# eldar/deepcut-cnn

Measured on AMD Instinct MI355X. Metric: images/sec, DeeperCut ResNet-152 FCN forward (prob+loc_pred+next_pred), whole node, higher is better.
Workload: dtype f32

## Files before the change

### deepcut-cnn_amd/csrc/c_api.cpp

```cpp
#include <hip/hip_runtime_api.h>

#include <cstdio>
#include <cstring>
#include <memory>
#include <string>
#include <vector>

#include "../../include/deepcut_hip.h"
#include "net.h"

using namespace dc;


namespace {
thread_local std::string g_err;
int fail(int code, const std::string& msg) {
  g_err = msg;
  return code;
}
template <typename F>
int guard(F&& f) {
  try {
    f();
    return DC_OK;
// ... 526 lines not shown
const char* dc_net_debug_info(dc_net* net) {
  if (!net) return nullptr;
  Net* n = N(net);
  int rc = guard([&] { n->text_buf = n->debug_info_text(); });
  return rc == DC_OK ? n->text_buf.c_str() : nullptr;
}

const char* dc_net_tune_report(dc_net* net) {
  if (!net) return nullptr;
  Net* n = N(net);
  int rc = guard([&] { n->text_buf = n->tune_report_text(); });
  return rc == DC_OK ? n->text_buf.c_str() : nullptr;
}
int dc_net_set_tile(dc_net* net, const char* signature, const char* tile) {
  REQUIRE(net);
  REQUIRE(signature);
  REQUIRE(tile);
  return guard([&] { N(net)->set_tile(signature, tile); });
}

int dc_conv_variant_count(void) { return dc::conv_num_variants(); }
const char* dc_conv_variant_name(int i) { return i >= 0 && i < dc::conv_num_variants() ? dc::conv_variant(i).name : nullptr; }
int dc_conv_variant_esize(int i) { return i >= 0 && i < dc::conv_num_variants() ? dc::conv_variant_esize(i) : 0; }
int dc_conv_bf16_variant_count(void) { return dc::conv_num_bf16_variants(); }
const char* dc_conv_bf16_variant_name(int i) {
  return i >= 0 && i < dc::conv_num_bf16_variants() ? dc::conv_variant(dc::kBf16Variant0 + i).name : nullptr;
}
int dc_wino_half_pack(const float* g, int cout, int cin, int rowscale, float* out, float* row_scale) {
  REQUIRE(g);
  REQUIRE(out);
  REQUIRE(row_scale);
  if (cout <= 0 || cin <= 0 || cout % 32 || cin % 16) return fail(DC_EINVAL, "dc_wino_half_pack: cout must be a multiple of 32, cin of 16");
  return guard([&] { dc::wino_half_pack_filters(g, cout, cin, rowscale != 0, out, row_scale); });
}

int dc_stream1x1_pack(const float* g, int cout, int k, float* out) {
  if (!g || !out) return fail(DC_EINVAL, "dc_stream1x1_pack: null pointer");
  if (cout <= 0 || k <= 0 || cout % 32 || k % 16) return fail(DC_EINVAL, "dc_stream1x1_pack: cout must be a multiple of 32, k of 16");
  return guard([&] { dc::stream1x1_pack_filters(g, cout, k, out); });
}

int dc_stream1x1f_pack(const float* g, int cout, int k, float* out) {
  if (!g || !out) return fail(DC_EINVAL, "dc_stream1x1f_pack: null pointer");
  if (cout <= 0 || k <= 0 || cout % 16 || k % 16) return fail(DC_EINVAL, "dc_stream1x1f_pack: cout and k must be multiples of 16");
  return guard([&] { dc::stream1x1f_pack_filters(g, cout, k, out); });
}

int dc_stem7x7_pack(const float* g, int c, float* out) {
  if (!g || !out) return fail(DC_EINVAL, "dc_stem7x7_pack: null pointer");
  if (c < 1 || c > 4) return fail(DC_EINVAL, "dc_stem7x7_pack: 1 to 4 input channels");
  return guard([&] { dc::stem7x7_pack_filters(g, c, out); });
}

namespace {
inline NetGroup* G(dc_group* g) { return reinterpret_cast<NetGroup*>(g); }
}
int dc_group_create(dc_net* const* nets, int n, dc_group** out) {
  REQUIRE(nets);
  REQUIRE(out);
  *out = nullptr;
  if (n <= 0) return fail(DC_EINVAL, "a group needs at least one net");
  return guard([&] {
    std::vector<Net*> m;
    for (int i = 0; i < n; ++i) m.push_back(N(nets[i]));
    *out = reinterpret_cast<dc_group*>(NetGroup::create(m));
  });
// ... 138 lines not shown
```

### deepcut-cnn_amd/csrc/kernels.h

```cpp
#pragma once
#include <cstddef>
#include <cstdint>
#include <string>

namespace dc {

constexpr int kMaxTaps = 32;

void dc_magic(unsigned d, unsigned (&mg)[2]);

enum ElemKind { kElemF32 = 0, kElemF16 = 1, kElemBF16 = 2 };
inline int elem_kind_size(int kind) { return kind == kElemF32 ? 4 : 2; }
inline const char* elem_kind_name(int kind) { return kind == kElemF16 ? "f16" : kind == kElemBF16 ? "bf16" : "f32"; }

constexpr int kMaxClasses = 4;
struct ConvClass {
  int nty, ntx, dy0, ddy, x0, ddx, Ktot, x_bias;
  int OH, OW, M;
  int tiles_m;
  unsigned div_ohw[2];
  unsigned div_ow[2];
  long w_off;
  long y_off;
};
// ... 71 lines not shown
};
struct ConvMultiArgs {
  ConvGemmParams p;
  ConvMultiTable t;
};
static_assert(sizeof(ConvMultiArgs) <= 4096, "HIP kernel arguments are limited to 4 KB");

struct ConvVariant {
  const char* name;
  int BM, BN, WR, WC, WK;
};
int conv_num_variants();
const ConvVariant& conv_variant(int i);
int conv_variant_bk(int i);
int conv_variant_esize(int i);
constexpr int kBf16Variant0 = 2000;
int conv_num_bf16_variants();
inline bool is_bf16_variant(int v) { return v >= kBf16Variant0 && v < kBf16Variant0 + conv_num_bf16_variants(); }
int conv_variant_ekind(int v);
bool conv_variant_exists(int v);
const int* conv_variants_of(int ekind, int* count);
int conv_variant_by_name(const char* name);
bool conv_variant_multiclass(int i);
long conv_grid(const ConvGemmParams& p, int variant);
int launch_conv_gemm(const ConvGemmParams& p, int variant, void* stream);
long prepare_conv_multi(ConvGemmParams& p, ConvMultiTable& table, int nprob, int variant);
bool conv_variant_multiproblem(int i);
int launch_conv_multi(const ConvMultiArgs& a, int variant, long grid, void* stream);

bool wino_eligible(const ConvGemmParams& p);
bool wino_same3x3(const ConvGemmParams& p);
ConvGemmParams wino_launch_params(const ConvGemmParams& p, long grid, int bty, int btx, int blocks_per_wg);
long wino_grid(const ConvGemmParams& p);
size_t wino_packed_floats(int Cout, int Cin);
void wino_pack_filters(const float* g, int Cout, int Cin, float* out);
bool wino_half_eligible(const ConvGemmParams& p);
long wino_half_grid(const ConvGemmParams& p);
size_t wino_half_packed_elems(int Cout, int Cin);
void wino_half_pack_filters(const float* g, int Cout, int Cin, bool rowscale, float* out, float* row_scale);
int launch_wino_half(const ConvGemmParams& p, void* stream);
bool stream1x1_eligible(const ConvGemmParams& p);
long stream1x1_grid(const ConvGemmParams& p);
size_t stream1x1_packed_elems(int Cout, int K);
void stream1x1_pack_filters(const float* g, int Cout, int K, float* out);
int launch_stream1x1(const ConvGemmParams& p, void* stream);
bool stream1x1f_eligible(const ConvGemmParams& p);
long stream1x1f_grid(const ConvGemmParams& p);
size_t stream1x1f_packed_elems(int Cout, int K);
void stream1x1f_pack_filters(const float* g, int Cout, int K, float* out);
int launch_stream1x1f(const ConvGemmParams& p, void* stream);
bool stem_ws_eligible(const ConvGemmParams& p);
long stem_ws_grid(const ConvGemmParams& p);
size_t stem_ws_packed_elems();
void stem_ws_pack_filters(const float* rowtap, float* out);
int launch_stem_ws(const ConvGemmParams& p, void* stream);
bool stem7x7_eligible(const ConvGemmParams& p);
long stem7x7_grid(const ConvGemmParams& p);
size_t stem7x7_packed_elems();
void stem7x7_pack_filters(const float* g, int C, float* out);
int launch_stem7x7(const ConvGemmParams& p, void* stream);
long stream1x1_prepare_multi(const ConvGemmParams& p, const ConvMultiTable& tb, int nprob);
int launch_stream1x1_multi(const ConvMultiArgs& a, void* stream);

constexpr int kWinoVariant = 1000;
constexpr int kWinoVariant16 = 1001;
constexpr int kWinoHalf = 1002;
constexpr int kStreamHalf = 1003;
constexpr int kStemHalf = 1004;
constexpr int kStreamFloat = 1005;
constexpr int kStemFloat = 1006;
constexpr int kFormVariant0 = kWinoVariant, kNumForms = 7;
enum FormGeometry { kForm3x3, kForm1x1, kFormStem };
struct ConvForm {
  int variant;
  const char *name, *label;
  int ekind, geometry, waves;
  const char* const* timing_slots;
  bool (*eligible)(const ConvGemmParams& p);
  long (*grid)(const ConvGemmParams& p);
  int (*launch)(const ConvGemmParams& p, void* stream);
  bool own_scale;
  bool merges;
  long (*prepare_multi)(const ConvGemmParams& p, const ConvMultiTable& tb, int nprob);
  int (*launch_multi)(const ConvMultiArgs& a, void* stream);
  int sibling;
  const char* env;
};
const ConvForm* conv_form(int variant);

const char* variant_name(int v);
int variant_by_name(const char* name);
std::string variant_kernel_label(int v);
long variant_grid(const ConvGemmParams& p, int v);
int launch_conv(const ConvGemmParams& p, int v, void* stream);


int launch_maxpool(const void* x, void* y, int ekind, int NB, int H, int W, int C, int OH, int OW, int k, int s,
                   int pad, void* stream);

int launch_eltwise(const void* x, const void* z, const float* a, const float* b, void* y, int ekind, long total, int C,
                   int relu, int sigmoid, void* stream);

int launch_crop(const void* x, void* y, int ekind, int NB, int H, int W, int C, int oh, int ow, int OH, int OW,
                void* stream);

int launch_nchw_to_nhwc(const float* src, void* dst, int ekind, int NB, int C, int H, int W, int CP, void* stream);
int launch_nhwc_to_nchw(const void* src, void* dst, int ekind, int NB, int C, int H, int W, int CP, int c0,
                        void* stream, int dst_esize = 4);
int launch_f32_to_f16(const float* src, void* dst, long n, void* stream);
int launch_f32_to_bf16(const float* src, void* dst, long n, void* stream);

int launch_part_select(const void* prob, int pcp, int pc0, const void* loc, int lcp, int lc0, int ekind, int NB, int H, int W, int J, float thr,
                       int radius, double scale, int max_det, unsigned long long* spill, int* counts, double* out, void* stream);
int launch_pairwise_decode(const void* next, int ncp, int nc0, int ekind, int NB, int H, int W, int E, double scale, int ndet,
                           const int* det , const double* mean, const double* stdev, double* out,
                           void* stream);

struct ImagePrepParams {
  const unsigned char* src;
// ... 49 lines not shown
```

### deepcut-cnn_amd/csrc/kernels.hip

```cpp
#include <hip/hip_runtime.h>

#include <algorithm>
#include <cstdlib>
#include <cstring>
#include <type_traits>
#include <vector>

#include "kernel_prims.h"
#include "kernels.h"

namespace dc {


#define DC_KARG_TOUCH(n0, n1, n2, n3, n4)                                                                                  \
  unsigned n0, n1, n2, n3, n4;                                                                                             \
  {                                                                                                                        \
    const auto* ka_ = __builtin_amdgcn_kernarg_segment_ptr();                                                              \
    asm volatile("s_load_dword %0, %5, 0x0\n\ts_load_dword %1, %5, 0x40\n\ts_load_dword %2, %5, 0x80\n\ts_load_dword %3, %5, 0xc0\n\t" \
                 "s_load_dword %4, %5, 0x100"                                                                              \
                 : "=&s"(n0), "=&s"(n1), "=&s"(n2), "=&s"(n3), "=&s"(n4)                                                     \
                 : "s"(ka_));                                                                                              \
  }
#define DC_KARG_HOLD(n0, n1, n2, n3, n4) asm volatile("" ::"s"(n0), "s"(n1), "s"(n2), "s"(n3), "s"(n4))
static_assert(sizeof(ConvGemmParams) >= 0x140, "DC_KARG_TOUCH reads five 64-byte lines of the argument block");
// ... 1259 lines not shown
  const long blk = mc_xcd_grid(p, rows, nprob, tn, wtot, atot);
  if (blk <= 0 || blk > 0x7fffffffL) return -1;
  {
    const int lgx = p.mc_lgx, lgy = 3 - lgx;
    const unsigned w0 = (unsigned)(tn >> lgx);
    dc_magic(std::max(w0, 1u), p.div_rw[0]);
    dc_magic(w0 + 1, p.div_rw[1]);
    for (int qy = 0; qy < 8; ++qy) {
      int run = 0;
      for (int c = 0; c < kMaxProblems; ++c) {
        if (c < nprob && qy < (8 >> lgx)) {
          run += (int)((((long)tb.prob[c].tiles_m * (qy + 1)) >> lgy) - (((long)tb.prob[c].tiles_m * qy) >> lgy));
          tb.end[qy][c] = run;
        } else {
          tb.end[qy][c] = 0x7fffffff;
        }
      }
    }
  }
  return blk;
}

int launch_conv_multi(const ConvMultiArgs& a, int variant, long grid, void* stream) {
  if (const ConvForm* f = conv_form(variant)) return f->launch_multi ? f->launch_multi(a, stream) : (int)hipErrorInvalidValue;
  if (!dc_variant_ok(variant) || !entry_of(variant).kernel_mp || a.p.nprob < 1 || grid <= 0) return (int)hipErrorInvalidValue;
  const VariantEntry& e = entry_of(variant);
  const int nt = e.v.WR * e.v.WC * e.v.WK * 64;
  hipLaunchKernelGGL(e.kernel_mp, dim3((unsigned)grid), dim3(nt), 0, (hipStream_t)stream, a);
  return (int)hipGetLastError();
}

namespace {
constexpr int WBTY = 4, WBTX = 8, WBN = 16, WKC = 32;
constexpr int WRH = 2 * WBTY + 2, WRW = 2 * WBTX + 2;
constexpr int WPSTR = WKC + 4;
constexpr int WPITCH = 672;
constexpr int WSTAGE = WRH * WPITCH + 8;
constexpr int WNTH = 512;
static_assert(WPITCH >= WRW * WPSTR && (2 * WPITCH) % 64 == 0 && WPSTR == 36, "conflict-free ds_read_b128 layout (see above)");
static_assert(WPITCH % 4 == 0 && WPSTR % 4 == 0 && WSTAGE % 4 == 0, "16-byte units");
__device__ __forceinline__ int wino_rowbase(int row) { return row * WPITCH; }
__device__ __forceinline__ f32x2 wlo(f32x4 v) { return __builtin_shufflevector(v, v, 0, 1); }
__device__ __forceinline__ f32x2 whi(f32x4 v) { return __builtin_shufflevector(v, v, 2, 3); }
}

template <int NG>
__global__ __launch_bounds__(WNTH * NG, 4) void wino_f23_kernel(const ConvGemmParams p) {
  constexpr int NTH = WNTH * NG;
  constexpr int WNLD = (WRH * WRW * (WKC / 4) + NTH - 1) / NTH;
  const long long t_entry = (long long)__builtin_amdgcn_s_memrealtime();
  DC_KARG_TOUCH(ka0, ka1, ka2, ka3, ka4);
  __shared__ __attribute__((aligned(16))) float stage[3][WSTAGE];
  float (*part)[4][2][2][4][64] = reinterpret_cast<float (*)[4][2][2][4][64]>(&stage[0][0]);
  static_assert(sizeof(float) * NG * 4 * 2 * 2 * 4 * 64 <= sizeof(stage), "partials must fit in the staging ring");
  static_assert(2 * sizeof(stage) <= 160 * 1024, "two workgroups per CU");
  const int t = threadIdx.x, lane = t & 63, wave = t >> 6;
  auto stamp = [&](int slot) {
    if (p.dbg && lane == 0) {
      long long* d = p.dbg + ((long)blockIdx.x * (8 * NG) + wave) * 12;
      d[slot] = (long long)__builtin_readcyclecounter();
      if (slot == 0) d[8] = t_entry, d[10] = (long long)__builtin_amdgcn_s_memrealtime();
      if (slot == 7) d[9] = (long long)__builtin_amdgcn_s_memrealtime();
    }
  };
  stamp(0);
  const int C = p.klen, H = p.x_rows, W = p.x_rowlen / p.klen;
  const int d = p.ddy;
  const int NBY = p.w_NBY, NBX = p.w_NBX;
  const int nblk = p.w_nblk;
  int lb = blockIdx.x;
  if (p.xcd_on) {
    const int g8 = gridDim.x >> 3, r8 = gridDim.x & 7, q = blockIdx.x & 7;
    lb = q * g8 + min(q, r8) + (blockIdx.x >> 3);
  }
  const int nt = dc_fastdiv(lb, p.w_div_nblk), blk = lb - nt * nblk;
  const int nph = dc_fastdiv(blk, p.w_div_nbyx), brem = blk - nph * (NBY * NBX);
  const int n = dc_fastdiv(nph, p.w_div_dd), ph = nph - n * (d * d);
  const int phy = dc_fastdiv(ph, p.w_div_d), phx = ph - phy * d;
  const int by = dc_fastdiv(brem, p.w_div_nbx), bx = brem - by * NBX;
  const int oy0 = 2 * WBTY * by - 1, ox0 = 2 * WBTX * bx - 1;
  DC_KARG_HOLD(ka0, ka1, ka2, ka3, ka4);
  const int kg = lane >> 4;
  const int grp = NG == 1 ? 0 : __builtin_amdgcn_readfirstlane(wave >> 3);
  const int i = wave & 3, tf = (wave >> 2) & 1;
  const int ra = i == 0 ? 0 : (i == 2 ? 2 : 1), rb = i == 0 ? 2 : (i == 1 ? 2 : (i == 2 ? 1 : 3));
  const float sb = i == 1 ? 1.f : -1.f;
  const __amdgpu_buffer_rsrc_t xr = dc_rsrc(reinterpret_cast<const float*>(p.x) + (long)n * p.x_img_stride, 0x7fffffffu);
  const __amdgpu_buffer_rsrc_t ur = dc_rsrc(p.w, 0x7fffffffu);
  unsigned gofs[WNLD];
  int sofs[WNLD];
#pragma unroll
  for (int q = 0; q < WNLD; ++q) {
    const int e = t + q * NTH;
    const int pix = e / (WKC / 4), cq = e % (WKC / 4);
    const int py = pix / WRW, px = pix % WRW;
    const int iy = phy + d * (oy0 + py), ix = phx + d * (ox0 + px);
    const bool ok = pix < WRH * WRW && oy0 + py >= 0 && ox0 + px >= 0 && iy < H && ix < W;
    gofs[q] = ok ? (unsigned)(iy * p.x_row_stride + ix * C + cq * 4) * 4u : kOOB;
    sofs[q] = (pix < WRH * WRW ? wino_rowbase(py) + px * WPSTR + cq * 4 : WSTAGE - 8 + (t & 1) * 4) >> 2;
  }
  const int r = (lane & 15) >> 3, c = lane & 7;
  const int ofs_a = wino_rowbase(2 * (2 * tf + r) + ra) + 2 * c * WPSTR + kg * 4;
  const int ofs_b = wino_rowbase(2 * (2 * tf + r) + rb) + 2 * c * WPSTR + kg * 4;
  f32x4 acc[4];
#pragma unroll
  for (int j = 0; j < 4; ++j) acc[j] = f32x4{0.f, 0.f, 0.f, 0.f};
  const unsigned uvo = ((unsigned)((nt * 4 + i) * (C / 16)) * (4 * 64 * 4) + (unsigned)lane * 4u) * 4u;
  f32x4 g[WNLD], b[2][4], da[4], db[4];
  auto gload = [&](int K) {
#pragma unroll
    for (int q = 0; q < WNLD; ++q) g[q] = dc_bload4(xr, gofs[q], (unsigned)(K * WKC * 4));
  };
  auto sstore = [&](int buf) {
#pragma unroll
    for (int q = 0; q < WNLD; ++q) reinterpret_cast<f32x4*>(&stage[buf][0])[sofs[q]] = g[q];
  };
  auto bload = [&](int slot, int k16) {
#pragma unroll
    for (int j = 0; j < 4; ++j) b[slot][j] = dc_bload4(ur, uvo + (unsigned)j * 1024u, (unsigned)k16 * 4096u);
  };
  auto lread = [&](int buf, int h) {
#pragma unroll
    for (int c4 = 0; c4 < 4; ++c4) {
      da[c4] = *reinterpret_cast<const f32x4*>(&stage[buf][ofs_a + c4 * WPSTR + h * 16]);
      db[c4] = *reinterpret_cast<const f32x4*>(&stage[buf][ofs_b + c4 * WPSTR + h * 16]);
    }
  };
  auto compute = [&](int bslot) {
    f32x2 tl[4], th[4];
    const f32x2 sb2 = {sb, sb};
#pragma unroll
    for (int c4 = 0; c4 < 4; ++c4) {
      tl[c4] = wlo(da[c4]) + sb2 * wlo(db[c4]);
      th[c4] = whi(da[c4]) + sb2 * whi(db[c4]);
    }
    f32x2 vl[4], vh[4];
// ... 59 lines not shown
    };
    for (int K0 = 0; K0 < NS; K0 += 6) {
      step(K0, std::integral_constant<int, 0>{}, std::integral_constant<int, 0>{});
      if (K0 + 1 < NS) step(K0 + 1, std::integral_constant<int, 1>{}, std::integral_constant<int, 1>{});
      if (K0 + 2 < NS) step(K0 + 2, std::integral_constant<int, 2>{}, std::integral_constant<int, 0>{});
      if (K0 + 3 < NS) step(K0 + 3, std::integral_constant<int, 0>{}, std::integral_constant<int, 1>{});
      if (K0 + 4 < NS) step(K0 + 4, std::integral_constant<int, 1>{}, std::integral_constant<int, 0>{});
      if (K0 + 5 < NS) step(K0 + 5, std::integral_constant<int, 2>{}, std::integral_constant<int, 1>{});
    }
  }
  stamp(4);
  __syncthreads();
#pragma unroll
  for (int r4 = 0; r4 < 4; ++r4) {
    part[grp][i][0][tf][r4][lane] = acc[0][r4] + acc[1][r4] + acc[2][r4];
    part[grp][i][1][tf][r4][lane] = acc[1][r4] - acc[2][r4] - acc[3][r4];
  }
  __syncthreads();
  stamp(5);
  const int a = (wave >> 1) & 1, bq = wave & 1;
  float* yb = reinterpret_cast<float*>(p.y);
  const float* rbp = reinterpret_cast<const float*>(p.resid);
  stamp(6);
#pragma unroll
  for (int rr = 0; rr < 4 / NG; ++rr) {
    const int r4 = NG == 1 ? rr : 2 * grp + rr;
    float p0 = part[0][0][bq][tf][r4][lane], p1 = part[0][1][bq][tf][r4][lane], p2 = part[0][2][bq][tf][r4][lane], p3 = part[0][3][bq][tf][r4][lane];
    if constexpr (NG == 2) {
      p0 += part[NG - 1][0][bq][tf][r4][lane], p1 += part[NG - 1][1][bq][tf][r4][lane];
      p2 += part[NG - 1][2][bq][tf][r4][lane], p3 += part[NG - 1][3][bq][tf][r4][lane];
    }
    float v = a == 0 ? p0 + p1 + p2 : p1 - p2 - p3;
    const int q = 4 * (lane >> 4) + r4;
    const int ty = by * WBTY + 2 * tf + (q >> 3), tx = bx * WBTX + (q & 7);
    const int oy = phy + d * (2 * ty + a), ox = phx + d * (2 * tx + bq);
    if (oy < p.OH && ox < p.OW) {
      const long off = (long)n * p.y_img_stride + (long)oy * p.y_row_stride + (long)ox * p.y_pix_stride + co;
      v = v * sc + sh;
      if (rbp) v += rbp[off];
      if (p.relu) v = fmaxf(v, 0.f);
      yb[off] = v;
    }
  }
  stamp(7);
}

bool wino_same3x3(const ConvGemmParams& p) {
  const int d = p.ddy;
  if (p.nty != 3 || p.ntx != 3 || p.sy != 1 || d < 1 || d > 4 || p.dy0 != -d) return false;
  const int C = p.klen;
  if (C <= 0) return false;
  if (p.sx != C || p.ddx != d * C || p.x0 != -d * C) return false;
  if (p.x_rowlen % C != 0 || p.x_row_stride != p.x_rowlen) return false;
  return p.OH == p.x_rows && p.OW == p.x_rowlen / C;
}

ConvGemmParams wino_launch_params(const ConvGemmParams& p, long grid, int bty, int btx, int blocks_per_wg) {
  ConvGemmParams q = p;
  q.xcd_on = xcd_map_on() && grid >= 16;
  const int d = p.ddy;
  q.w_TY = ((p.OH + d - 1) / d + 1) / 2, q.w_TX = ((p.OW + d - 1) / d + 1) / 2;
  q.w_NBY = (q.w_TY + bty - 1) / bty, q.w_NBX = (q.w_TX + btx - 1) / btx;
  q.w_nblk = p.NB * d * d * q.w_NBY * q.w_NBX;
  dc_magic((unsigned)((q.w_nblk + blocks_per_wg - 1) / blocks_per_wg), q.w_div_nblk);
  dc_magic((unsigned)(q.w_NBY * q.w_NBX), q.w_div_nbyx);
  dc_magic((unsigned)(d * d), q.w_div_dd);
  dc_magic((unsigned)d, q.w_div_d);
  dc_magic((unsigned)q.w_NBX, q.w_div_nbx);
  return q;
}

bool wino_eligible(const ConvGemmParams& p) {
  if (p.esize != 4 || !wino_same3x3(p)) return false;
  const int C = p.klen;
  if (C % WKC != 0 || p.Cout % WBN != 0 || p.sigmoid_ch != 0) return false;
  if ((long long)p.x_rows * p.x_row_stride * 4 >= 0x7fffffffLL || (long long)wino_packed_floats(p.Cout, C) * 4 >= 0x7fffffffLL) return false;
  return true;
}

long wino_grid(const ConvGemmParams& p) {
  const int d = p.ddy;
  const int TY = ((p.OH + d - 1) / d + 1) / 2, TX = ((p.OW + d - 1) / d + 1) / 2;
  return (long)p.NB * d * d * ((TY + WBTY - 1) / WBTY) * ((TX + WBTX - 1) / WBTX) * (p.Cout / WBN);
}

size_t wino_packed_floats(int Cout, int Cin) { return (size_t)16 * Cout * Cin; }

void wino_pack_filters(const float* g, int Cout, int Cin, float* out) {
  static const double G[4][3] = {{1, 0, 0}, {.5, .5, .5}, {.5, -.5, .5}, {0, 0, 1}};
  for (int co = 0; co < Cout; ++co)
    for (int ci = 0; ci < Cin; ++ci) {
      const float* w = g + ((size_t)co * Cin + ci) * 9;
      double tmp[4][3], U[4][4];
      for (int a = 0; a < 4; ++a)
        for (int b = 0; b < 3; ++b) tmp[a][b] = G[a][0] * w[b] + G[a][1] * w[3 + b] + G[a][2] * w[6 + b];
      for (int a = 0; a < 4; ++a)
        for (int b = 0; b < 4; ++b) U[a][b] = tmp[a][0] * G[b][0] + tmp[a][1] * G[b][1] + tmp[a][2] * G[b][2];
      const int nt = co / 16, col = co % 16, k16 = ci / 16, kg = (ci % 16) / 4, s = ci % 4;
      const int lane = kg * 16 + col;
      for (int i = 0; i < 4; ++i)
        for (int j = 0; j < 4; ++j)
          out[(((((size_t)nt * 4 + i) * (Cin / 16) + k16) * 4 + j) * 64 + lane) * 4 + s] = (float)U[i][j];
    }
}

template <int NG>
static int launch_wino_f23(const ConvGemmParams& p, void* stream) {
  if (p.esize != 4 || !wino_eligible(p)) return (int)hipErrorInvalidValue;
  const long grid = wino_grid(p);
  if (grid <= 0) return 0;
  if (grid > 0x7fffffffL) return (int)hipErrorInvalidValue;
  hipLaunchKernelGGL(wino_f23_kernel<NG>, dim3((unsigned)grid), dim3(NG * WNTH), 0, (hipStream_t)stream, wino_launch_params(p, grid, WBTY, WBTX, 1));
  return (int)hipGetLastError();
}

static const char* const kWinoSlots[7] = {"index setup", "first loads issued", "two stages in LDS", "K loop", "partials to LDS + barrier",
                                          "inverse transform + epilogue constants", "shortcut + stores"};
static const char* const kStreamSlots[7] = {"prologue requests issued", "first stage + filters landed", "the first D steps", "the other steps",
                                            "drain", "-", "exit"};
static constexpr ConvForm kForms[kNumForms] = {
    {kWinoVariant, "wino_f23", "wino_f23<4x8x16>", kElemF32, kForm3x3, 8, kWinoSlots, wino_eligible, wino_grid, launch_wino_f23<1>,
     false, false, nullptr, nullptr, kWinoVariant16, "DC_WINOGRAD"},
    {kWinoVariant16, "wino_f23_w16", "wino_f23<4x8x16_w16>", kElemF32, kForm3x3, 16, kWinoSlots, wino_eligible, wino_grid, launch_wino_f23<2>,
     false, false, nullptr, nullptr, kWinoVariant, "DC_WINOGRAD"},
    {kWinoHalf, "wino_h23", "wino_h23<2x4x8x64>", kElemF16, kForm3x3, 8, kWinoSlots, wino_half_eligible, wino_half_grid, launch_wino_half,
     true, true, nullptr, nullptr, -1, "DC_WINOGRAD"},
    {kStreamHalf, "ws1x1", "ws1x1<32xN>", kElemF16, kForm1x1, 4, kStreamSlots, stream1x1_eligible, stream1x1_grid, launch_stream1x1,
     false, true, stream1x1_prepare_multi, launch_stream1x1_multi, -1, "DC_STREAM1X1"},
    {kStemHalf, "stem7x7", "stem7x7<8x64>", kElemF16, kFormStem, 4, kWinoSlots, stem7x7_eligible, stem7x7_grid, launch_stem7x7,
     false, false, nullptr, nullptr, -1, "DC_STEM"},
    {kStreamFloat, "ws1x1f", "ws1x1f<16xN>", kElemF32, kForm1x1, 4, kStreamSlots, stream1x1f_eligible, stream1x1f_grid, launch_stream1x1f,
     false, true, nullptr, nullptr, -1, "DC_STREAM1X1"},
    {kStemFloat, "ws7x7f", "ws7x7f<16x64>", kElemF32, kFormStem, 4, kStreamSlots, stem_ws_eligible, stem_ws_grid, launch_stem_ws,
     false, true, nullptr, nullptr, -1, "DC_STEM"},
};

static constexpr bool forms_in_variant_order() {
  for (int i = 0; i < kNumForms; ++i)
    if (kForms[i].variant != kFormVariant0 + i) return false;
  return true;
}
static_assert(forms_in_variant_order(), "row i of kForms is variant kFormVariant0 + i");

const ConvForm* conv_form(int variant) {
  return variant >= kFormVariant0 && variant < kFormVariant0 + kNumForms ? &kForms[variant - kFormVariant0] : nullptr;
}

const char* variant_name(int v) {
  const ConvForm* f = conv_form(v);
  return f ? f->name : conv_variant(v).name;
}
int variant_by_name(const char* name) {
  for (const ConvForm& f : kForms)
    if (std::strcmp(name, f.name) == 0) return f.variant;
  return conv_variant_by_name(name);
}
std::string variant_kernel_label(int v) {
  const ConvForm* f = conv_form(v);
  return f ? std::string(f->label) : std::string("conv_gemm<") + conv_variant(v).name + ">";
}
long variant_grid(const ConvGemmParams& p, int v) {
  const ConvForm* f = conv_form(v);
  return f ? f->grid(p) : conv_grid(p, v);
}
int launch_conv(const ConvGemmParams& p, int v, void* stream) {
  const ConvForm* f = conv_form(v);
  return f ? f->launch(p, stream) : launch_conv_gemm(p, v, stream);
}

template <typename F>
static int dc_by_kind(int ekind, F&& f) {
  if (ekind == kElemF16) return f((_Float16*)nullptr);
  if (ekind == kElemBF16) return f((__bf16*)nullptr);
  return f((float*)nullptr);
}
// ... 652 lines not shown
```

### deepcut-cnn_amd/csrc/net_tune.cpp

```cpp
#include <unistd.h>

#include "net_internal.h"

namespace dc {

void load_tune_cache_locked(ModelShared& shared) {
  if (shared.tune_file_loaded) return;
  shared.tune_file_loaded = true;
  const char* cache_path = std::getenv("DC_TUNE_CACHE");
  if (!cache_path || !*cache_path) return;
  FILE* f = std::fopen(cache_path, "r");
  if (!f) return;
  std::string line;
  int ch;
  auto take = [&]() {
    const size_t sp = line.find_last_of(' ');
    if (sp != std::string::npos && sp > 0 && sp + 1 < line.size()) {
      const std::string key = line.substr(0, sp), vname = line.substr(sp + 1);
      const int v = variant_by_name(vname.c_str());
      if (v >= 0 && !shared.tune_cache.count(key)) shared.tune_cache[key] = v;
    }
    line.clear();
  };
  while ((ch = std::fgetc(f)) != EOF) {
// ... 35 lines not shown
    }
  } ev_guard{e0, e1};
  HIPCHECK(hipEventCreate(&e0));
  HIPCHECK(hipEventCreate(&e1));
  const int reps = 5;
  auto key_of = [&](const Launch& l) { return tune_key(l); };
  auto burst_ms = [&](const Launch& trial) {
    run_launch(trial, stream);
    float ms = 1e30f;
    for (int t2 = 0; t2 < 2; ++t2) {
      HIPCHECK(hipEventRecord(e0, (hipStream_t)stream));
      for (int r = 0; r < reps; ++r) run_launch(trial, stream);
      HIPCHECK(hipEventRecord(e1, (hipStream_t)stream));
      HIPCHECK(hipEventSynchronize(e1));
      float m2 = 0;
      HIPCHECK(hipEventElapsedTime(&m2, e0, e1));
      ms = std::min(ms, m2);
    }
    return ms;
  };
  std::map<std::string, std::vector<std::pair<float, int>>> timed;
  for (auto& l : plan) {
    if (l.kind != Launch::CONV) continue;
    const std::string key = key_of(l);
    if (tune_cache_.count(key)) continue;
    timed_any = true;
    std::vector<std::pair<float, int>>& c = timed[key];
    int ncand = 0;
    const int* cand = conv_variants_of(l.cg.ekind, &ncand);
    std::vector<int> vs(cand, cand + ncand);
    for (int v = kFormVariant0; v < kFormVariant0 + kNumForms; ++v) vs.push_back(v);
    for (int v : vs) {
      if (!l.takes_tile(v)) continue;
      Launch trial = l;
      trial.variant = v;
      c.push_back({burst_ms(trial), v});
    }
    std::sort(c.begin(), c.end());
    tune_cache_[key] = c.empty() ? l.variant : c.front().second;
    shared->tune_timings[key] = c;
  }
  if (timed_any && env_int("DC_TUNE_INSITU", 1) != 0) {
    std::map<std::string, std::vector<int>> shortlist;
    size_t rounds = 0;
    for (auto& kv : timed) {
      std::vector<int> sl;
      for (auto& c : kv.second)
        if (sl.size() < 4 && c.first <= kv.second.front().first * 1.12f) sl.push_back(c.second);
      if (sl.size() >= 2) {
        rounds = std::max(rounds, sl.size());
        shortlist[kv.first] = sl;
      }
    }
    if (rounds) {
      std::vector<int> idx;
      std::vector<std::string> keys;
      for (size_t i = 0; i < plan.size(); ++i) {
        if (plan[i].kind != Launch::CONV) continue;
        std::string k = key_of(plan[i]);
        if (shortlist.count(k)) idx.push_back((int)i), keys.push_back(k);
      }
      std::vector<hipEvent_t> ev(2 * idx.size(), nullptr);
      std::vector<Launch> saved = plan;
      struct Restore {
        std::vector<Launch>& plan;
        std::vector<Launch>& saved;
// ... 172 lines not shown
```

### deepcut-cnn_amd/python/caffe/__init__.py

```python
from .pycaffe import Net, NetGroup, Comm, Blob, Layer, choose_streams, pinned_empty, lpt_schedule, set_mode_cpu, set_mode_gpu, set_device, device_count, canvas_size, check_boxes, member_canvas, conv_variants, conv_variants_bf16, wino_half_pack, stream1x1_pack, stream1x1f_pack, stem7x7_pack, lib_path
from .pycaffe import TRAIN, TEST, DeepcutError

__version__ = "1.0.0-rc3+deepcut_hip"
```

### deepcut-cnn_amd/python/caffe/pycaffe.py

```python
import ctypes as C
import os
import sys
from collections import OrderedDict

import numpy as np

TRAIN = 0
TEST = 1

_HERE = os.path.dirname(os.path.abspath(__file__))
_LIB_CANDIDATES = [
    os.environ.get("DEEPCUT_HIP_LIB", ""),
    os.path.normpath(os.path.join(_HERE, "..", "..", "lib", "libdeepcut_hip.so")),
]


class DeepcutError(RuntimeError):

    def __init__(self, code, msg):
        RuntimeError.__init__(self, msg)
        self.code = code


def lib_path():
# ... 83 lines not shown
        "dc_group_destroy": (ci, [vp]),
        "dc_group_size": (ci, [vp]),
        "dc_group_set_lanes": (ci, [vp, ci]),
        "dc_group_forward_batch": (ci, [vp, C.POINTER(vp), C.POINTER(ci), C.POINTER(ci), C.POINTER(ci), ci, C.POINTER(vp), C.POINTER(vp),
                                        C.POINTER(vp), vp]),
        "dc_group_forward_images": (ci, [vp, C.POINTER(vp), C.POINTER(ci), C.POINTER(ci), C.POINTER(ci), C.POINTER(C.c_double), ci,
                                         C.POINTER(vp), C.POINTER(vp), C.POINTER(vp), C.POINTER(vp), vp]),
        "dc_group_forward_boxes": (ci, [vp, vp, ci, ci, ci, vp, vp, ci, C.POINTER(C.c_double), ci, ci, C.POINTER(vp), C.POINTER(vp),
                                        C.POINTER(vp), C.POINTER(vp), vp]),
        "dc_group_plan_text": (cp, [vp]),
        "dc_group_profile_text": (cp, [vp, ci]),
        "dc_group_tune_report": (cp, [vp]),
        "dc_group_set_tile": (ci, [vp, cp, cp]),
        "dc_group_stats": (ci, [vp, C.POINTER(C.c_longlong), ci]),
        "dc_group_flops": (ci, [vp, C.POINTER(C.c_double)]),
        "dc_net_forward_host_async": (ci, [vp, vp, ci, ci, ci, vp, vp, vp]),
        "dc_host_alloc": (ci, [C.c_size_t, C.POINTER(vp)]),
        "dc_host_free": (ci, [vp]),
        "dc_nets_choose_streams": (ci, [C.POINTER(vp), ci, ci, ci, C.POINTER(C.c_double), C.POINTER(C.c_double)]),
        "dc_net_stream": (ci, [vp, C.POINTER(vp)]),
        "dc_comm_create": (ci, [ci, C.POINTER(ci), ci, C.POINTER(vp)]),
        "dc_comm_destroy": (ci, [vp]),
        "dc_comm_transport": (ci, [vp]),
        "dc_forward_batch": (ci, [vp, C.POINTER(vp), ci, C.POINTER(vp), C.POINTER(ci * 2), ci, C.POINTER(vp), C.POINTER(vp), C.POINTER(vp)]),
        "dc_comm_item_executor": (ci, [vp, ci]),
        "dc_comm_root_maps": (ci, [vp, ci, C.POINTER(vp), C.POINTER(vp), C.POINTER(vp), C.POINTER(ci)]),
        "dc_lpt_schedule": (ci, [C.POINTER(C.c_double), ci, ci, C.POINTER(ci)]),
        "dc_conv_variant_count": (ci, []),
        "dc_conv_variant_name": (cp, [ci]),
        "dc_conv_variant_esize": (ci, [ci]),
        "dc_conv_bf16_variant_count": (ci, []),
        "dc_conv_bf16_variant_name": (cp, [ci]),
        "dc_wino_half_pack": (ci, [C.c_void_p, ci, ci, ci, C.c_void_p, C.c_void_p]),
        "dc_stream1x1_pack": (ci, [C.c_void_p, ci, ci, C.c_void_p]),
        "dc_stem7x7_pack": (ci, [C.c_void_p, ci, C.c_void_p]),
        "dc_stream1x1f_pack": (ci, [C.c_void_p, ci, ci, C.c_void_p]),
    }
    for name, (res, args) in sig.items():
        fn = getattr(lib, name)
        fn.restype = res
        fn.argtypes = args
    return lib, sorted(sig)


_lib, EXPORTED_SYMBOLS = _load()


def _check(rc):
    if rc != 0:
        raise DeepcutError(rc, (_lib.dc_last_error() or b"").decode())


def set_mode_cpu():
    _check(_lib.dc_set_mode(0))


def set_mode_gpu():
    _check(_lib.dc_set_mode(1))


def set_device(device_id):
    _check(_lib.dc_set_device(int(device_id)))


def device_count():
    return _lib.dc_device_count()


_DTYPES = {"f32": 0, "float32": 0, "f16": 1, "float16": 1, "bf16": 2, "bfloat16": 2}


def conv_variants():
    return [((_lib.dc_conv_variant_name(i) or b"").decode(), _lib.dc_conv_variant_esize(i)) for i in range(_lib.dc_conv_variant_count())]


def conv_variants_bf16():
    return [(_lib.dc_conv_bf16_variant_name(i) or b"").decode() for i in range(_lib.dc_conv_bf16_variant_count())]


def stream1x1_pack(g):
    g = np.ascontiguousarray(g, np.float32)
    cout, k = g.shape[0], int(np.prod(g.shape[1:]))
    out = np.empty((cout // 32, k // 16, 64, 8), np.float32)
    _check(_lib.dc_stream1x1_pack(g.ctypes.data_as(C.c_void_p), cout, k, out.ctypes.data_as(C.c_void_p)))
    return out


def stream1x1f_pack(g):
    g = np.ascontiguousarray(g, np.float32)
    cout, k = g.shape[0], int(np.prod(g.shape[1:]))
    out = np.empty((cout // 16, k // 16, 64, 4), np.float32)
    _check(_lib.dc_stream1x1f_pack(g.ctypes.data_as(C.c_void_p), cout, k, out.ctypes.data_as(C.c_void_p)))
    return out


def stem7x7_pack(g):
    g = np.ascontiguousarray(g, np.float32)
    if g.ndim != 4 or g.shape[0] != 64 or g.shape[2:] != (7, 7):
        raise ValueError("stem7x7_pack: g must be [64, c, 7, 7]")
    out = np.empty((2, 7, 2, 64, 8), np.float32)
    _check(_lib.dc_stem7x7_pack(g.ctypes.data_as(C.c_void_p), g.shape[1], out.ctypes.data_as(C.c_void_p)))
    return out


def wino_half_pack(g, rowscale=True):
    g = np.ascontiguousarray(g, dtype=np.float32)
    cout, cin = g.shape[:2]
    out = np.empty((cout // 32, 4, cin // 16, 4, 64, 8), np.float32)
    rs = np.empty(cout, np.float32)
    _check(_lib.dc_wino_half_pack(g.ctypes.data_as(C.c_void_p), cout, cin, 1 if rowscale else 0, out.ctypes.data_as(C.c_void_p), rs.ctypes.data_as(C.c_void_p)))
# ... 846 lines not shown
```

### deepcut-cnn_amd/python/deepcut_tools/tuning.py

```python


_WINO_SIBLING = {"wino_f23": "wino_f23_w16", "wino_f23_w16": "wino_f23"}


def tune_in_flight(nets, run, top=6, margin=1.20, min_gain=0.01, reps=3, max_candidates=2, log=None):
    runs = [0]

    def measure():
        run()
        runs[0] += reps + 1
        return min(run() for _ in range(reps))

    before = incumbent = measure()
    report = nets[0].tune_report()
    have = [set(s["signature"] for s in n.tune_report()) for n in nets[1:]]
    ranked, skipped = [], 0
    for sig in report:
        if len(sig["timed"]) < 2 and sig["tile"] in _WINO_SIBLING:
            sig = dict(sig, timed=[(sig["tile"], 15.0), (_WINO_SIBLING[sig["tile"]], 15.0)])
        if len(sig["timed"]) < 2:
            skipped += 1
            continue
        if any(sig["signature"] not in h for h in have):
            skipped += 1
            continue
        alone = dict(sig["timed"])
        ranked.append((alone.get(sig["tile"], sig["timed"][0][1]) * sig["launches"], sig))
    ranked.sort(key=lambda t: -t[0])
    def put(signature, tile):
        for n in nets:
            n.set_tile(signature, tile)

    changed = []
    for _share, sig in ranked[:top]:
        best_alone = sig["timed"][0][1]
# ... 27 lines not shown
```

### include/deepcut_hip.h

```cpp
#ifndef DEEPCUT_HIP_H_
#define DEEPCUT_HIP_H_

#include <stddef.h>
#include <stdint.h>

#ifdef __cplusplus
extern "C" {
#endif

#define DC_OK 0
#define DC_EINVAL (-1)
#define DC_EIO (-2)
#define DC_ESHAPE (-3)
#define DC_EUNSUP (-4)
#define DC_EDEVICE (-5)
#define DC_ENOCPU (-6)

#define DC_MODE_CPU 0
#define DC_MODE_GPU 1
#define DC_PHASE_TRAIN 0
#define DC_PHASE_TEST 1

#define DC_OPT_FUSE 1
#define DC_OPT_HIPGRAPH 2
// ... 83 lines not shown

int dc_net_forward_boxes(dc_net* net, const unsigned char* image, int height, int width, int is_device, const int* boxes, const double* scales,
                         int n, int canvas_h, int canvas_w, float* prob, float* loc_pred, float* next_pred, double* pose, void* stream);

int dc_net_detect_parts(dc_net* net, double scale, float threshold, int radius, int max_det, int* counts, double* dets);
int dc_net_decode_pairwise(dc_net* net, double scale, int ndet, const int* detections, const double* mean,
                           const double* stdev, double* out);


int dc_net_flops(dc_net* net, double* flops);
int dc_net_num_launches(dc_net* net);
#define DC_STAT_LOWERINGS 0
#define DC_STAT_GRAPH_INSTANTIATIONS 1
#define DC_STAT_PLAN_HITS 2
#define DC_STAT_AUTOTUNE_RUNS 3
#define DC_STAT_BUFFER_GROWTHS 4
#define DC_STAT_REPACKS 5
#define DC_STAT_CACHED_PLANS 6
#define DC_NUM_STATS 7
int dc_net_stats(dc_net* net, long long* out, int n);
int dc_net_reserve(dc_net* net, int n, int h, int w);
int dc_net_device(dc_net* net);
const char* dc_net_plan_text(dc_net* net);
const char* dc_net_profile_text(dc_net* net, int iters);
const char* dc_net_debug_info(dc_net* net);
const char* dc_net_tune_report(dc_net* net);
int dc_net_set_tile(dc_net* net, const char* signature, const char* tile);
int dc_conv_variant_count(void);
const char* dc_conv_variant_name(int i);
int dc_conv_variant_esize(int i);
int dc_conv_bf16_variant_count(void);
const char* dc_conv_bf16_variant_name(int i);
int dc_wino_half_pack(const float* g, int cout, int cin, int rowscale, float* out, float* row_scale);

int dc_stream1x1_pack(const float* g, int cout, int k, float* out);
int dc_stem7x7_pack(const float* g, int c, float* out);
int dc_stream1x1f_pack(const float* g, int cout, int k, float* out);

typedef struct dc_group dc_group;
int dc_group_create(dc_net* const* nets, int n, dc_group** out);
int dc_group_destroy(dc_group* group);
int dc_group_size(dc_group* group);
int dc_group_set_lanes(dc_group* group, int lanes);
int dc_group_forward_batch(dc_group* group, const float* const* inputs, const int* n, const int* h, const int* w, int is_device,
                           float* const* prob, float* const* loc_pred, float* const* next_pred, void* stream);
int dc_group_forward_images(dc_group* group, const unsigned char* const* images, const int* n, const int* height, const int* width,
                            const double* scale, int is_device, float* const* prob, float* const* loc_pred, float* const* next_pred,
                            double* const* pose, void* stream);
int dc_group_forward_boxes(dc_group* group, const unsigned char* image, int height, int width, int is_device, const int* boxes,
                           const double* scales, int n, const double* pyramid_scales, int canvas_h, int canvas_w, float* const* prob,
                           float* const* loc_pred, float* const* next_pred, double* const* pose, void* stream);
const char* dc_group_plan_text(dc_group* group);
const char* dc_group_profile_text(dc_group* group, int iters);
const char* dc_group_tune_report(dc_group* group);
int dc_group_set_tile(dc_group* group, const char* signature, const char* tile);
#define DC_GSTAT_MERGES 0
#define DC_GSTAT_GRAPH_INSTANTIATIONS 1
#define DC_GSTAT_AUTOTUNE_RUNS 2
#define DC_GSTAT_PLAN_HITS 3
#define DC_GSTAT_LAUNCHES 4
#define DC_GSTAT_MULTI_LAUNCHES 5
#define DC_GSTAT_LANES 6
#define DC_NUM_GSTATS 7
int dc_group_stats(dc_group* group, long long* out, int n);
int dc_group_flops(dc_group* group, double* out);

// ... 18 lines not shown
```

Baseline: 517.6.

## Add 5x6-tile Winograd F(2,3) block shape as autotuned variant

Templates the Winograd F(2,3) kernel on a tile geometry and adds a 5x6 output-tile block (15 tiles per fragment, new LDS pitch) alongside the existing 4x8 block. The autotuner considers the new variants only for layers where they produce fewer blocks, cutting wasted edge tiles on feature-map sizes that divide poorly by 4x8. The cost is one idle lane per 16-lane group, an extra bounds predicate in the epilogue, and more variants to tune.

```diff
diff --git a/deepcut-cnn_amd/csrc/c_api.cpp b/deepcut-cnn_amd/csrc/c_api.cpp
--- a/deepcut-cnn_amd/csrc/c_api.cpp
+++ b/deepcut-cnn_amd/csrc/c_api.cpp
@@ -582,6 +582,15 @@
   REQUIRE(row_scale);
   if (cout <= 0 || cin <= 0 || cout % 32 || cin % 16) return fail(DC_EINVAL, "dc_wino_half_pack: cout must be a multiple of 32, cin of 16");
   return guard([&] { dc::wino_half_pack_filters(g, cout, cin, rowscale != 0, out, row_scale); });
+}
+
+int dc_wino_blocks(const char* tile, int tiles_y, int tiles_x) {
+  if (!tile || tiles_y < 1 || tiles_x < 1) return -1;
+  try {
+    return (int)dc::wino_form_blocks(dc::variant_by_name(tile), tiles_y, tiles_x);
+  } catch (...) {
+    return -1;
+  }
 }
 
 int dc_stream1x1_pack(const float* g, int cout, int k, float* out) {
diff --git a/deepcut-cnn_amd/csrc/kernels.h b/deepcut-cnn_amd/csrc/kernels.h
--- a/deepcut-cnn_amd/csrc/kernels.h
+++ b/deepcut-cnn_amd/csrc/kernels.h
@@ -127,6 +127,8 @@
 bool wino_same3x3(const ConvGemmParams& p);
 ConvGemmParams wino_launch_params(const ConvGemmParams& p, long grid, int bty, int btx, int blocks_per_wg);
 long wino_grid(const ConvGemmParams& p);
+long wino_blocks(int TY, int TX, int bty, int btx);
+long wino_form_blocks(int variant, int TY, int TX);
 size_t wino_packed_floats(int Cout, int Cin);
 void wino_pack_filters(const float* g, int Cout, int Cin, float* out);
 bool wino_half_eligible(const ConvGemmParams& p);
@@ -164,7 +166,9 @@
 constexpr int kStemHalf = 1004;
 constexpr int kStreamFloat = 1005;
 constexpr int kStemFloat = 1006;
-constexpr int kFormVariant0 = kWinoVariant, kNumForms = 7;
+constexpr int kWinoVariant56 = 1007;
+constexpr int kWinoVariant56x16 = 1008;
+constexpr int kFormVariant0 = kWinoVariant, kNumForms = 9;
 enum FormGeometry { kForm3x3, kForm1x1, kFormStem };
 struct ConvForm {
   int variant;
@@ -180,6 +184,7 @@
   int (*launch_multi)(const ConvMultiArgs& a, void* stream);
   int sibling;
   const char* env;
+  bool (*offered)(const ConvGemmParams& p) = nullptr;
 };
 const ConvForm* conv_form(int variant);
 
diff --git a/deepcut-cnn_amd/csrc/kernels.hip b/deepcut-cnn_amd/csrc/kernels.hip
--- a/deepcut-cnn_amd/csrc/kernels.hip
+++ b/deepcut-cnn_amd/csrc/kernels.hip
@@ -1315,21 +1315,47 @@
 
 namespace {
 constexpr int WBTY = 4, WBTX = 8, WBN = 16, WKC = 32;
-constexpr int WRH = 2 * WBTY + 2, WRW = 2 * WBTX + 2;
 constexpr int WPSTR = WKC + 4;
 constexpr int WPITCH = 672;
-constexpr int WSTAGE = WRH * WPITCH + 8;
 constexpr int WNTH = 512;
-static_assert(WPITCH >= WRW * WPSTR && (2 * WPITCH) % 64 == 0 && WPSTR == 36, "conflict-free ds_read_b128 layout (see above)");
-static_assert(WPITCH % 4 == 0 && WPSTR % 4 == 0 && WSTAGE % 4 == 0, "16-byte units");
-__device__ __forceinline__ int wino_rowbase(int row) { return row * WPITCH; }
+template <int FR_, int FC_, bool SIDE_, int PITCH_>
+struct WinoGeom {
+  static constexpr int FR = FR_, FC = FC_, NT = FR_ * FC_, PITCH = PITCH_;
+  static constexpr bool SIDE = SIDE_;
+  static constexpr int BTY = SIDE_ ? FR_ : 2 * FR_, BTX = SIDE_ ? 2 * FC_ : FC_;
+  static constexpr int RH = 2 * BTY + 2, RW = 2 * BTX + 2;
+  static constexpr int STAGE = RH * PITCH_ + 8;
+  static constexpr int frow(int tf) { return SIDE_ ? 0 : FR_ * tf; }
+  static constexpr int fcol(int tf) { return SIDE_ ? FC_ * tf : 0; }
+  static constexpr int trow(int tf, int q) { return frow(tf) + q / FC_; }
+  static constexpr int tcol(int tf, int q) { return fcol(tf) + q % FC_; }
+  static constexpr bool conflict_free() {
+    for (int tf = 0; tf < 2; ++tf)
+      for (int flip = 0; flip < 2; ++flip) {
+        bool seen[16] = {};
+        for (int q = 0; q < NT; ++q) {
+          const int slot = ((2 * trow(tf, q) * PITCH_ + 2 * tcol(tf, q) * WPSTR) / 4 + ((q >= 4 && q < 12) != (flip != 0) ? 1 : 0)) & 15;
+          if (seen[slot]) return false;
+          seen[slot] = true;
+        }
+      }
+    return true;
+  }
+  static_assert(NT <= 16 && PITCH_ >= RW * WPSTR && WPSTR == 36 && conflict_free(), "conflict-free ds_read_b128 layout (see above)");
+  static_assert(PITCH_ % 4 == 0 && WPSTR % 4 == 0 && STAGE % 4 == 0, "16-byte units");
+};
+using WinoG48 = WinoGeom<WBTY / 2, WBTX, false, WPITCH>;
+using WinoG56 = WinoGeom<5, 3, true, 524>;
+static_assert(WinoG48::BTY == 4 && WinoG48::BTX == 8 && WinoG48::RH == 10 && WinoG48::RW == 18, "the 4 x 8 block");
+static_assert(WinoG56::BTY == 5 && WinoG56::BTX == 6 && WinoG56::RH == 12 && WinoG56::RW == 14, "the 5 x 6 block");
 __device__ __forceinline__ f32x2 wlo(f32x4 v) { return __builtin_shufflevector(v, v, 0, 1); }
 __device__ __forceinline__ f32x2 whi(f32x4 v) { return __builtin_shufflevector(v, v, 2, 3); }
 }
 
-template <int NG>
+template <int NG, class G>
 __global__ __launch_bounds__(WNTH * NG, 4) void wino_f23_kernel(const ConvGemmParams p) {
   constexpr int NTH = WNTH * NG;
+  constexpr int BTY = G::BTY, BTX = G::BTX, WRH = G::RH, WRW = G::RW, PITCH = G::PITCH, WSTAGE = G::STAGE;
   constexpr int WNLD = (WRH * WRW * (WKC / 4) + NTH - 1) / NTH;
   const long long t_entry = (long long)__builtin_amdgcn_s_memrealtime();
   DC_KARG_TOUCH(ka0, ka1, ka2, ka3, ka4);
@@ -1361,7 +1387,7 @@
   const int n = dc_fastdiv(nph, p.w_div_dd), ph = nph - n * (d * d);
   const int phy = dc_fastdiv(ph, p.w_div_d), phx = ph - phy * d;
   const int by = dc_fastdiv(brem, p.w_div_nbx), bx = brem - by * NBX;
-  const int oy0 = 2 * WBTY * by - 1, ox0 = 2 * WBTX * bx - 1;
+  const int oy0 = 2 * BTY * by - 1, ox0 = 2 * BTX * bx - 1;
   DC_KARG_HOLD(ka0, ka1, ka2, ka3, ka4);
   const int kg = lane >> 4;
   const int grp = NG == 1 ? 0 : __builtin_amdgcn_readfirstlane(wave >> 3);
@@ -1380,11 +1406,12 @@
     const int iy = phy + d * (oy0 + py), ix = phx + d * (ox0 + px);
     const bool ok = pix < WRH * WRW && oy0 + py >= 0 && ox0 + px >= 0 && iy < H && ix < W;
     gofs[q] = ok ? (unsigned)(iy * p.x_row_stride + ix * C + cq * 4) * 4u : kOOB;
-    sofs[q] = (pix < WRH * WRW ? wino_rowbase(py) + px * WPSTR + cq * 4 : WSTAGE - 8 + (t & 1) * 4) >> 2;
-  }
-  const int r = (lane & 15) >> 3, c = lane & 7;
-  const int ofs_a = wino_rowbase(2 * (2 * tf + r) + ra) + 2 * c * WPSTR + kg * 4;
-  const int ofs_b = wino_rowbase(2 * (2 * tf + r) + rb) + 2 * c * WPSTR + kg * 4;
+    sofs[q] = (pix < WRH * WRW ? py * PITCH + px * WPSTR + cq * 4 : WSTAGE - 8 + (t & 1) * 4) >> 2;
+  }
+  const int qt = G::NT < 16 ? min(lane & 15, G::NT - 1) : lane & 15;
+  const int r = qt / G::FC, c = G::fcol(tf) + qt % G::FC;
+  const int ofs_a = (2 * (G::frow(tf) + r) + ra) * PITCH + 2 * c * WPSTR + kg * 4;
+  const int ofs_b = (2 * (G::frow(tf) + r) + rb) * PITCH + 2 * c * WPSTR + kg * 4;
   f32x4 acc[4];
 #pragma unroll
   for (int j = 0; j < 4; ++j) acc[j] = f32x4{0.f, 0.f, 0.f, 0.f};
@@ -1510,9 +1537,9 @@
     }
     float v = a == 0 ? p0 + p1 + p2 : p1 - p2 - p3;
     const int q = 4 * (lane >> 4) + r4;
-    const int ty = by * WBTY + 2 * tf + (q >> 3), tx = bx * WBTX + (q & 7);
+    const int ty = by * BTY + G::frow(tf) + q / G::FC, tx = bx * BTX + G::fcol(tf) + q % G::FC;
     const int oy = phy + d * (2 * ty + a), ox = phx + d * (2 * tx + bq);
-    if (oy < p.OH && ox < p.OW) {
+    if ((G::NT == 16 || q < G::NT) && oy < p.OH && ox < p.OW) {
       const long off = (long)n * p.y_img_stride + (long)oy * p.y_row_stride + (long)ox * p.y_pix_stride + co;
       v = v * sc + sh;
       if (rbp) v += rbp[off];
@@ -1556,11 +1583,17 @@
   return true;
 }
 
-long wino_grid(const ConvGemmParams& p) {
+long wino_blocks(int TY, int TX, int bty, int btx) { return (long)((TY + bty - 1) / bty) * ((TX + btx - 1) / btx); }
+
+template <class G>
+static long wino_grid_of(const ConvGemmParams& p) {
   const int d = p.ddy;
   const int TY = ((p.OH + d - 1) / d + 1) / 2, TX = ((p.OW + d - 1) / d + 1) / 2;
-  return (long)p.NB * d * d * ((TY + WBTY - 1) / WBTY) * ((TX + WBTX - 1) / WBTX) * (p.Cout / WBN);
-}
+  return (long)p.NB * d * d * wino_blocks(TY, TX, G::BTY, G::BTX) * (p.Cout / WBN);
+}
+long wino_grid(const ConvGemmParams& p) { return wino_grid_of<WinoG48>(p); }
+
+static bool wino_fewer_blocks(const ConvGemmParams& p) { return wino_grid_of<WinoG56>(p) < wino_grid_of<WinoG48>(p); }
 
 size_t wino_packed_floats(int Cout, int Cin) { return (size_t)16 * Cout * Cin; }
 
@@ -1582,13 +1615,13 @@
     }
 }
 
-template <int NG>
+template <int NG, class G>
 static int launch_wino_f23(const ConvGemmParams& p, void* stream) {
   if (p.esize != 4 || !wino_eligible(p)) return (int)hipErrorInvalidValue;
-  const long grid = wino_grid(p);
+  const long grid = wino_grid_of<G>(p);
   if (grid <= 0) return 0;
   if (grid > 0x7fffffffL) return (int)hipErrorInvalidValue;
-  hipLaunchKernelGGL(wino_f23_kernel<NG>, dim3((unsigned)grid), dim3(NG * WNTH), 0, (hipStream_t)stream, wino_launch_params(p, grid, WBTY, WBTX, 1));
+  hipLaunchKernelGGL((wino_f23_kernel<NG, G>), dim3((unsigned)grid), dim3(NG * WNTH), 0, (hipStream_t)stream, wino_launch_params(p, grid, G::BTY, G::BTX, 1));
   return (int)hipGetLastError();
 }
 
@@ -1597,9 +1630,9 @@
 static const char* const kStreamSlots[7] = {"prologue requests issued", "first stage + filters landed", "the first D steps", "the other steps",
                                             "drain", "-", "exit"};
 static constexpr ConvForm kForms[kNumForms] = {
-    {kWinoVariant, "wino_f23", "wino_f23<4x8x16>", kElemF32, kForm3x3, 8, kWinoSlots, wino_eligible, wino_grid, launch_wino_f23<1>,
+    {kWinoVariant, "wino_f23", "wino_f23<4x8x16>", kElemF32, kForm3x3, 8, kWinoSlots, wino_eligible, wino_grid, launch_wino_f23<1, WinoG48>,
      false, false, nullptr, nullptr, kWinoVariant16, "DC_WINOGRAD"},
-    {kWinoVariant16, "wino_f23_w16", "wino_f23<4x8x16_w16>", kElemF32, kForm3x3, 16, kWinoSlots, wino_eligible, wino_grid, launch_wino_f23<2>,
+    {kWinoVariant16, "wino_f23_w16", "wino_f23<4x8x16_w16>", kElemF32, kForm3x3, 16, kWinoSlots, wino_eligible, wino_grid, launch_wino_f23<2, WinoG48>,
      false, false, nullptr, nullptr, kWinoVariant, "DC_WINOGRAD"},
     {kWinoHalf, "wino_h23", "wino_h23<2x4x8x64>", kElemF16, kForm3x3, 8, kWinoSlots, wino_half_eligible, wino_half_grid, launch_wino_half,
      true, true, nullptr, nullptr, -1, "DC_WINOGRAD"},
@@ -1611,6 +1644,10 @@
      false, true, nullptr, nullptr, -1, "DC_STREAM1X1"},
     {kStemFloat, "ws7x7f", "ws7x7f<16x64>", kElemF32, kFormStem, 4, kStreamSlots, stem_ws_eligible, stem_ws_grid, launch_stem_ws,
      false, true, nullptr, nullptr, -1, "DC_STEM"},
+    {kWinoVariant56, "wino_f23_5x6", "wino_f23<5x6x16>", kElemF32, kForm3x3, 8, kWinoSlots, wino_eligible, wino_grid_of<WinoG56>, launch_wino_f23<1, WinoG56>,
+     false, false, nullptr, nullptr, kWinoVariant56x16, "DC_WINOGRAD", wino_fewer_blocks},
+    {kWinoVariant56x16, "wino_f23_5x6_w16", "wino_f23<5x6x16_w16>", kElemF32, kForm3x3, 16, kWinoSlots, wino_eligible, wino_grid_of<WinoG56>, launch_wino_f23<2, WinoG56>,
+     false, false, nullptr, nullptr, kWinoVariant56, "DC_WINOGRAD", wino_fewer_blocks},
 };
 
 static constexpr bool forms_in_variant_order() {
@@ -1619,6 +1656,12 @@
   return true;
 }
 static_assert(forms_in_variant_order(), "row i of kForms is variant kFormVariant0 + i");
+
+long wino_form_blocks(int variant, int TY, int TX) {
+  if (variant == kWinoVariant || variant == kWinoVariant16) return wino_blocks(TY, TX, WinoG48::BTY, WinoG48::BTX);
+  if (variant == kWinoVariant56 || variant == kWinoVariant56x16) return wino_blocks(TY, TX, WinoG56::BTY, WinoG56::BTX);
+  return -1;
+}
 
 const ConvForm* conv_form(int variant) {
   return variant >= kFormVariant0 && variant < kFormVariant0 + kNumForms ? &kForms[variant - kFormVariant0] : nullptr;
diff --git a/deepcut-cnn_amd/csrc/net_tune.cpp b/deepcut-cnn_amd/csrc/net_tune.cpp
--- a/deepcut-cnn_amd/csrc/net_tune.cpp
+++ b/deepcut-cnn_amd/csrc/net_tune.cpp
@@ -91,6 +91,8 @@
     for (int v = kFormVariant0; v < kFormVariant0 + kNumForms; ++v) vs.push_back(v);
     for (int v : vs) {
       if (!l.takes_tile(v)) continue;
+      if (const ConvForm* f = conv_form(v))
+        if (f->offered && !f->offered(l.cg)) continue;
       Launch trial = l;
       trial.variant = v;
       c.push_back({burst_ms(trial), v});
diff --git a/deepcut-cnn_amd/python/caffe/__init__.py b/deepcut-cnn_amd/python/caffe/__init__.py
--- a/deepcut-cnn_amd/python/caffe/__init__.py
+++ b/deepcut-cnn_amd/python/caffe/__init__.py
@@ -1,4 +1,4 @@
-from .pycaffe import Net, NetGroup, Comm, Blob, Layer, choose_streams, pinned_empty, lpt_schedule, set_mode_cpu, set_mode_gpu, set_device, device_count, canvas_size, check_boxes, member_canvas, conv_variants, conv_variants_bf16, wino_half_pack, stream1x1_pack, stream1x1f_pack, stem7x7_pack, lib_path
+from .pycaffe import Net, NetGroup, Comm, Blob, Layer, choose_streams, pinned_empty, lpt_schedule, set_mode_cpu, set_mode_gpu, set_device, device_count, canvas_size, check_boxes, member_canvas, conv_variants, conv_variants_bf16, wino_half_pack, wino_blocks, stream1x1_pack, stream1x1f_pack, stem7x7_pack, lib_path
 from .pycaffe import TRAIN, TEST, DeepcutError
 
 __version__ = "1.0.0-rc3+deepcut_hip"
diff --git a/deepcut-cnn_amd/python/caffe/pycaffe.py b/deepcut-cnn_amd/python/caffe/pycaffe.py
--- a/deepcut-cnn_amd/python/caffe/pycaffe.py
+++ b/deepcut-cnn_amd/python/caffe/pycaffe.py
@@ -139,6 +139,7 @@
         "dc_conv_bf16_variant_count": (ci, []),
         "dc_conv_bf16_variant_name": (cp, [ci]),
         "dc_wino_half_pack": (ci, [C.c_void_p, ci, ci, ci, C.c_void_p, C.c_void_p]),
+        "dc_wino_blocks": (ci, [cp, ci, ci]),
         "dc_stream1x1_pack": (ci, [C.c_void_p, ci, ci, C.c_void_p]),
         "dc_stem7x7_pack": (ci, [C.c_void_p, ci, C.c_void_p]),
         "dc_stream1x1f_pack": (ci, [C.c_void_p, ci, ci, C.c_void_p]),
@@ -183,6 +184,10 @@
 
 def conv_variants_bf16():
     return [(_lib.dc_conv_bf16_variant_name(i) or b"").decode() for i in range(_lib.dc_conv_bf16_variant_count())]
+
+
+def wino_blocks(tile, tiles_y, tiles_x):
+    return _lib.dc_wino_blocks(tile.encode(), int(tiles_y), int(tiles_x))
 
 
 def stream1x1_pack(g):
diff --git a/deepcut-cnn_amd/python/deepcut_tools/tuning.py b/deepcut-cnn_amd/python/deepcut_tools/tuning.py
--- a/deepcut-cnn_amd/python/deepcut_tools/tuning.py
+++ b/deepcut-cnn_amd/python/deepcut_tools/tuning.py
@@ -1,6 +1,6 @@
 
 
-_WINO_SIBLING = {"wino_f23": "wino_f23_w16", "wino_f23_w16": "wino_f23"}
+_WINO_SIBLING = {"wino_f23": "wino_f23_w16", "wino_f23_w16": "wino_f23", "wino_f23_5x6": "wino_f23_5x6_w16", "wino_f23_5x6_w16": "wino_f23_5x6"}
 
 
 def tune_in_flight(nets, run, top=6, margin=1.20, min_gain=0.01, reps=3, max_candidates=2, log=None):
diff --git a/include/deepcut_hip.h b/include/deepcut_hip.h
--- a/include/deepcut_hip.h
+++ b/include/deepcut_hip.h
@@ -139,6 +139,7 @@
 int dc_conv_bf16_variant_count(void);
 const char* dc_conv_bf16_variant_name(int i);
 int dc_wino_half_pack(const float* g, int cout, int cin, int rowscale, float* out, float* row_scale);
+int dc_wino_blocks(const char* tile, int tiles_y, int tiles_x);
 
 int dc_stream1x1_pack(const float* g, int cout, int k, float* out);
 int dc_stem7x7_pack(const float* g, int c, float* out);
```

After: 531.7 (median of 6 runs). 1.03x the previous value.
